# miloknowles/adaptive-stereo-icra-2021

Measured on AMD Instinct MI355X. Metric: stereo pairs/sec (fwd+adapt-step), KITTI 1242x375 D=192, higher is better.
Workload: dtype f32; 1 GPU; KITTI-2015 1242x375, maxdisp 192, k=4 (Dc=12, 24x78 cost volume), forward + one online-adapt step (train-mode BN, monodepth loss, clip 1.0, Adam lr 5e-5); pairs_per_gpu=4, global_batch=4, parallelism=dp1 (per-replica BatchNorm statistics, one flat RCCL gradient all-reduce), kernels=all hand-written HIP (no MIOpen/rocBLAS on the path)

## Files before the change

### adaptive-stereo-icra-2021_amd/adaptive_stereo/_native.py

```python
import ctypes
import os

import torch

_HERE = os.path.dirname(os.path.abspath(__file__))
LIB_PATH = os.path.join(_HERE, "libadaptive_stereo_hip.so")
BUILD_HINT = "build it with: make -C %s" % os.path.join(os.path.dirname(_HERE), "csrc")

c_int, c_float, c_i64, c_vp = ctypes.c_int, ctypes.c_float, ctypes.c_int64, ctypes.c_void_p


class Pcl(ctypes.Structure):
  _fields_ = [(n, ctypes.c_int32) for n in ("B", "D", "H", "W", "pd", "ph", "pw")]

  def numel(self):
    return self.B * (self.D + 2 * self.pd) * (self.H + 2 * self.ph) * (self.W + 2 * self.pw) * 32

  def voxels(self):
    return self.B * self.D * self.H * self.W

  def key(self):
    return (self.B, self.D, self.H, self.W, self.pd, self.ph, self.pw)


# ... 79 lines not shown
                                      c_vp, c_vp, c_vp, c_vp]),
  "as_conv32_wino_bwd_filter": (c_int, [c_vp, c_vp, _P(Pcl), _P(ConvShape), c_vp, c_vp, c_int, c_vp, c_vp]),
  "as_conv32_wino_bwd_parts": (c_int, []),
  "as_conv32_wino_bwd_workspace": (c_i64, []),
  "as_conv32_wino_bwd_generation": (c_int, [c_int]),
  "as_conv32_wino_bwd": (c_int, [c_vp, _P(Pcl), c_vp, c_vp, _P(Pcl), _P(ConvShape), c_vp, c_vp, c_vp, c_vp, c_vp, c_float, c_vp,
                                 c_vp, c_vp, c_vp, c_vp, c_vp, c_vp, c_vp, c_int, c_vp, c_vp, c_vp]),
  "as_conv32_wino_bwd_fused_parts": (c_int, []),
  "as_conv32_wino_bwd_fused_workspace": (c_i64, []),
  "as_conv32_wino_bwd_fused": (c_int, [c_vp, _P(Pcl), c_vp, c_vp, _P(Pcl), _P(ConvShape), c_vp, c_vp, c_vp, c_vp, c_vp, c_float, c_vp,
                                       c_vp, c_vp, c_vp, c_vp, c_vp, c_vp, c_int, c_vp, c_vp, c_vp]),
  "as_conv3d_wgrad_lds_assignment": (c_int, [c_int, c_int, c_int, c_vp, c_vp, c_vp]),
  "as_conv32_s2_enable": (c_int, [c_int]),
  "as_conv4_s2_enable": (c_int, [c_int]),
  "as_conv4_s2_ok": (c_int, [_P(Pcl), _P(Pcl), _P(ConvShape)]),
  "as_conv32_s2_fwd_ok": (c_int, [_P(Pcl), _P(Pcl), _P(ConvShape)]),
  "as_conv32_s2_dgrad_ok": (c_int, [_P(Pcl), _P(Pcl)]),
  "as_conv32_wgrad_segments": (c_int, [_P(Pcl), _P(Pcl), _P(ConvShape)]),
  "as_refine_out_ok": (c_int, [_P(Pcl)]),
  "as_refine_out_fwd": (c_int, [c_vp, c_vp, c_vp, c_vp, c_float, c_vp, _P(Pcl), c_vp, c_vp, c_vp, c_int, c_vp, c_vp]),
  "as_conv32_bwd_fused_ok": (c_int, [_P(Pcl), _P(Pcl), _P(ConvShape)]),
  "as_conv32_bwd_fused_parts": (c_int, []),
  "as_conv32_bwd_fused_workspace": (c_i64, []),
  "as_conv32_bwd_fused": (c_int, [c_vp, _P(Pcl), c_vp, c_vp, _P(Pcl), _P(ConvShape), c_vp, c_vp, c_vp, c_vp, c_vp, c_float, c_vp, c_vp,
                                  c_vp, c_vp, c_vp, c_vp, c_vp, c_int, c_vp, c_vp, c_vp]),
  "as_conv32_bnbwd_parts": (c_int, [_P(Pcl), _P(Pcl), _P(ConvShape)]),
  "as_conv32_fwd_bnbwd": (c_int, [c_vp, _P(Pcl), c_vp, c_vp, _P(Pcl), _P(ConvShape), c_vp, c_vp, c_vp, c_vp, c_vp, c_float,
                                  c_vp, c_vp]),
  "as_agg3d_ok": (c_int, [_P(Pcl)]),
  "as_agg3d_parts": (c_int, [_P(Pcl)]),
  "as_agg3d_plan": (c_int, [_P(Pcl), c_vp]),
  "as_agg3d_fwd": (c_int, [c_vp, _P(Pcl), c_vp, c_vp, c_vp, c_vp, _P(BnMerge), c_vp, c_vp, c_int, c_vp, c_vp, c_float, c_vp, c_vp,
                           c_vp, c_vp]),
  "as_trunk_parts": (c_int, [_P(Pcl), c_int]),
  "as_trunk_fwd": (c_int, [c_vp, c_vp, _P(TrunkBn), c_vp, _P(Pcl), c_int, c_vp, c_vp, c_float, c_vp, c_vp, c_vp, c_vp, c_vp]),
  "as_trunk_finish_fwd": (c_int, [c_vp, _P(Pcl), c_vp, c_vp, c_int, c_int, _P(c_vp), _P(c_vp), c_float, c_vp]),
  "as_trunk_begin_bwd": (c_int, [c_vp, c_vp, c_int, _P(Pcl), c_vp, c_vp]),
  "as_trunk_bwd_workspace": (c_i64, [_P(Pcl), c_int]),
  "as_trunk_bwd": (c_int, [c_vp, c_vp, c_vp, c_vp, c_int, c_vp, c_vp, c_vp, c_vp, c_vp, c_vp, c_vp, c_vp, _P(Pcl), c_int, c_float,
                           c_vp, c_vp, c_int, c_vp, c_vp]),
  "as_trunk_finish_bwd": (c_int, [c_vp, c_int, c_int, _P(c_vp), _P(c_vp), c_int, c_vp]),
  "as_agg_tail_ok": (c_int, [_P(Pcl)]),
  "as_agg_tail_fwd_positions": (c_int, [_P(Pcl)]),
  "as_agg_tail_fwd": (c_int, [c_vp, _P(Pcl), c_vp, c_vp, _P(BnMerge), c_vp, c_vp, c_vp, c_float, c_vp, c_vp, c_vp, c_vp, c_vp]),
  "as_conv3d_out_fwd": (c_int, [c_vp, _P(Pcl), c_vp, c_vp, c_vp, c_vp]),
  "as_conv3d_out_bwd_workspace": (c_i64, [_P(Pcl)]),
  "as_conv3d_out_bwd": (c_int, [c_vp, c_vp, _P(Pcl), c_vp, c_vp, c_vp, c_vp, c_int, c_vp, c_vp]),
  "as_conv32to1_fwd": (c_int, [c_vp, _P(Pcl), _P(ConvShape), c_vp, c_vp, c_vp, c_int, c_vp, c_vp]),
  "as_conv32to1_bwd_workspace": (c_i64, [_P(Pcl), _P(ConvShape)]),
  "as_conv32to1_bwd": (c_int, [c_vp, c_vp, _P(Pcl), _P(ConvShape), c_vp, c_vp, c_vp, c_vp, c_int, c_vp, c_vp]),
  "as_pcl4_numel": (c_i64, [_P(Pcl)]),
  "as_pack_in4": (c_int, [c_vp, c_vp, c_int, c_vp, _P(Pcl), c_vp]),
  "as_conv4_pack_weights": (c_int, [c_vp, c_int, c_vp, _P(ConvShape), c_vp]),
  "as_conv4_wgrad_bnapply_ok": (c_int, [_P(Pcl), _P(Pcl), _P(ConvShape)]),
  "as_conv4_wgrad_bnapply_proj": (c_int, [c_vp, _P(Pcl), c_vp, c_vp, _P(Pcl), _P(ConvShape), c_int, c_vp, c_vp, c_vp, c_vp, c_float,
                                          c_vp, c_vp, c_vp, c_vp, c_int, c_vp, c_vp]),
  "as_tap_gather": (c_int, [c_vp, c_vp, c_vp, c_int, c_int, c_int, c_vp]),
  "as_conv4_wgrad_bnapply": (c_int, [c_vp, _P(Pcl), c_vp, c_vp, _P(Pcl), _P(ConvShape), c_int, c_vp, c_vp, c_vp, c_vp, c_float,
                                     c_vp, c_vp, c_vp, c_int, c_vp, c_vp]),
  "as_conv4_stat_parts": (c_int, [_P(Pcl), _P(Pcl), _P(ConvShape)]),
  "as_conv4_fwd": (c_int, [c_vp, _P(Pcl), c_vp, c_vp, c_vp, _P(Pcl), _P(ConvShape), c_int, c_vp, c_vp, c_float,
                           c_vp, c_vp, c_vp, c_vp]),
  "as_conv4_wgrad_workspace": (c_i64, [_P(Pcl), _P(ConvShape)]),
  "as_conv4_wgrad": (c_int, [c_vp, _P(Pcl), c_vp, _P(Pcl), _P(ConvShape), c_int, c_vp, c_vp, c_int, c_vp, c_vp]),
  "as_softargmax_fwd": (c_int, [c_vp, c_int, c_int, c_int, c_int, c_vp, c_vp, c_vp, c_vp]),
  "as_softargmax_bwd": (c_int, [c_vp, c_vp, c_vp, c_int, c_int, c_int, c_int, c_vp, c_vp]),
# ... 152 lines not shown
```

### adaptive-stereo-icra-2021_amd/adaptive_stereo/hip_ops.py

```python
import torch

from . import _native as nat
from ._native import Pcl, ConvShape, call, ptr, stream, f32c

LEAKY_SLOPE = 0.2
BN_EPS = 1e-5
BN_MOMENTUM = 0.1

CONV3D_333 = ConvShape(3, 3, 3, 1, 1, 1, 1, 1)

_DIRECT_GRADS = True


def set_direct_grad_accumulation(flag: bool):
  global _DIRECT_GRADS
  _DIRECT_GRADS = bool(flag)


def grad_sinks(params):
  if not (_DIRECT_GRADS and torch.is_grad_enabled()):
    return None
  out = []
  for p in params:
    g = getattr(p, "grad", None)
# ... 673 lines not shown

def set_agg3d(flag: bool):
  global _AGG3D
  prev, _AGG3D = _AGG3D, bool(flag)
  return prev


def set_bwd_fused(flag: bool):
  global _BWD_FUSED
  prev, _BWD_FUSED = _BWD_FUSED, bool(flag)
  return prev


_AGG_MERGE_MAX = 512
_TAIL_BWD = True


def set_tail_bwd(flag: bool):
  global _TAIL_BWD
  prev, _TAIL_BWD = _TAIL_BWD, bool(flag)
  return prev


def set_agg_tail(flag: bool):
  global _AGG_TAIL
  prev, _AGG_TAIL = _AGG_TAIL, bool(flag)
  return prev


def agg3d_ok(g: Pcl):
  return _AGG3D and nat.load().as_agg3d_ok(g) == 1


class PendingBn(object):

  def __init__(self, stats: StatParts, gamma, beta, running_mean, running_var):
    self.stats, self.gamma, self.beta, self.rm, self.rv = stats, gamma, beta, running_mean, running_var
    self.state = BnState(gamma.device)
    st = self.state
    self.block = nat.BnMerge(ptr(stats.mean), ptr(stats.m2), ptr(stats.cnt), ptr(gamma), ptr(beta), ptr(running_mean),
                             ptr(running_var), ptr(st.mean), ptr(st.invstd), ptr(st.scale), ptr(st.shift), stats.nparts,
                             BN_MOMENTUM, BN_EPS)

  def finalize(self):
    st = self.state
    with _rmw(self.rm):
      call("as_bn_finalize", ptr(self.stats.mean), ptr(self.stats.m2), ptr(self.stats.cnt), self.stats.nparts, ptr(self.gamma),
           ptr(self.beta), ptr(self.rm), ptr(self.rv), BN_MOMENTUM, BN_EPS, ptr(st.mean), ptr(st.invstd), ptr(st.scale),
           ptr(st.shift), stream())
    return st


def agg3d(x, g: Pcl, packed_w, bias, z=None, in_state=None, in_bn=None, a_out=None, epilogue=0, ep_state=None, stats=None):
  z = z if z is not None else POOL.get(g, x.device)
  sm, s2, sc = (stats.mean, stats.m2, stats.cnt) if stats is not None else (None, None, None)
  with _rmw(in_bn.rm if in_bn is not None else None):
    call("as_agg3d_fwd", ptr(x), g, ptr(packed_w), ptr(bias), ptr(in_state.scale) if in_state is not None else None,
         ptr(in_state.shift) if in_state is not None else None, in_bn.block if in_bn is not None else None, ptr(a_out), ptr(z),
         int(epilogue), ptr(ep_state.scale) if ep_state is not None else None,
         ptr(ep_state.shift) if ep_state is not None else None, LEAKY_SLOPE, ptr(sm), ptr(s2), ptr(sc), stream())
  return z


class CostAggregationFn(torch.autograd.Function):

  @staticmethod
# ... 87 lines not shown
    ctx.mark_non_differentiable(argmax, fcs)
    ctx.set_materialize_grads(False)
    return logits, pred, argmax, fcs

  @staticmethod
  def backward(ctx, g_logits_in, g_pred, _g_argmax, _g_fcs):
    logits, *params = ctx.saved_tensors
    g = ctx.g
    dev = logits.device
    B, D, H, W = logits.shape
    lib = nat.load()
    xs, zs, sts = ctx.xs, ctx.zs, ctx.sts

    g_pred, g_logits_in = f32c(g_pred), f32c(g_logits_in)
    grads = [None] * 18
    w_out = params[16]
    sinks = ctx.sinks
    g_a = POOL.get(g, dev)
    g_wout, g_bout, acc = _grad_dest(_sink(sinks, 16), _sink(sinks, 17), w_out.shape, (1,), dev)
    if not acc:
      grads[16], grads[17] = g_wout, g_bout
    if _TAIL_BWD and lib.as_agg_tail_bwd_ok(g) == 1:
      ws = _empty(lib.as_agg_tail_bwd_workspace(g), dev)
      call("as_agg_tail_bwd", ptr(logits), ptr(g_pred), ptr(g_logits_in), ptr(xs[4]), g, ptr(w_out), ptr(g_a), ptr(g_wout),
           ptr(g_bout), acc, ptr(ws), stream())
    else:
      g_logits = torch.empty_like(logits)
      call("as_softargmax_bwd", ptr(logits), ptr(g_pred), ptr(g_logits_in), B, D, H, W, ptr(g_logits), stream())
      ws = _empty(lib.as_conv3d_out_bwd_workspace(g), dev)
      call("as_conv3d_out_bwd", ptr(g_logits), ptr(xs[4]), g, ptr(w_out), ptr(g_a), ptr(g_wout), ptr(g_bout), acc, ptr(ws),
           stream())

    need_feat = ctx.needs_input_grad[0] or ctx.needs_input_grad[1]
    for l in range(3, -1, -1):
      w, b, gamma, beta = params[4 * l:4 * l + 4]
      g_x, dW, db, g_gamma, g_beta, _ = block_backward(g_a, xs[l], zs[l], sts[l], w, gamma, g, CONV3D_333, ctx.train,
                                                       False, l > 0 or need_feat,
                                                       sinks[4 * l:4 * l + 4] if sinks is not None else None)
      grads[4 * l:4 * l + 4] = [dW, db, g_gamma, g_beta]
      POOL.put(g_a, g); POOL.put(zs[l], g); POOL.put(xs[l + 1], g)
      g_a = g_x
    g_fl = g_fr = None
    if need_feat:
      g_fl = torch.empty(B, 32, H, W, dtype=torch.float32, device=dev)
      g_fr = torch.empty_like(g_fl)
      call("as_cost_volume_bwd", ptr(g_a), ptr(g_fl), ptr(g_fr), g, stream())
      POOL.put(g_a, g)
    POOL.put(xs[0], g)
    ctx.xs = ctx.zs = ctx.sts = None
    return (g_fl, g_fr, None, None, None, None, None) + tuple(grads)


CONV5_S2 = ConvShape(1, 5, 5, 0, 2, 2, 1, 2)


def _down(n):
  return (n - 1) // 2 + 1


_TRUNK = True


def set_trunk(flag: bool):
  global _TRUNK
  prev, _TRUNK = _TRUNK, bool(flag)
  return prev


def trunk_enabled():
  return _TRUNK and _BN_SYNC is None

# ... 677 lines not shown
```

### adaptive-stereo-icra-2021_amd/csrc/agg3d.hip

```cpp
#include "as_common.h"
#include "conv_epilogue.h"
#include "agg3d.h"
#include "bn_merge.h"

#ifndef AGG_WRING
#define AGG_WRING 9
#endif

struct Agg3dArgs {
  const float* x;
  const float* wq;
  const float* in_scale;
  const float* in_shift;
  float* a_out;
  EpilogueArgs ep;
  BnMergeDev in_bn;
  PclDev g;
  int tiles_per_plane, npos, run, groups, slot_bytes;
  int seg_len, nseg, units, per_xcd;
  unsigned wp_magic;
  int strips, Ws, tiles_per_strip;
};

typedef __attribute__((address_space(3))) void* lds_as3_t;

__device__ inline void agg_dma_1kb(const float* sbase, unsigned voff, unsigned m0) {
  asm volatile("s_mov_b32 m0, %0\n\ts_nop 0\n\tglobal_load_lds_dwordx4 %1, %2"
               :: "s"(m0), "v"(voff), "s"(sbase) : "memory", "m0");
}
template <int IMM> __device__ inline void agg_store_imm(float* sbase, unsigned voff, float v) {
  asm volatile("global_store_dword %0, %1, %2 offset:%3" :: "v"(voff), "v"(v), "s"(sbase), "n"(IMM) : "memory");
}
#define AGG_ROW_IMM(r) ((((r) & 3) + 8 * ((r) >> 2)) * 128)
#define AGG_FOR_ROWS(M) M(0) M(1) M(2) M(3) M(4) M(5) M(6) M(7) M(8) M(9) M(10) M(11) M(12) M(13) M(14) M(15)

__device__ inline f32x4 agg_chunk(const char* slot, int v, int h, int q) {
  return *reinterpret_cast<const f32x4*>(slot + v * 128 + (((4 * h + q) ^ ((v >> 1) & 7)) << 4));
}
typedef unsigned agg_u32x4 __attribute__((ext_vector_type(4)));
__device__ inline void agg_load_w(f32x4 (&r)[4], __amdgpu_buffer_rsrc_t rsrc, unsigned lane_bytes, int tap) {
#pragma unroll
  for (int q = 0; q < 4; ++q) {
    const agg_u32x4 v = __builtin_amdgcn_raw_buffer_load_b128(rsrc, lane_bytes + q * 1024, tap * 4096, 0);
    r[q] = __builtin_bit_cast(f32x4, v);
  }
}

__device__ inline int agg_div_wp(int pos, unsigned magic) { return (int)__umulhi((unsigned)pos, magic); }

__device__ inline void agg_issue_plane(const Agg3dArgs& p, int b, int q, int pos0, long plane_vox, unsigned lds0, int wave,
                                       unsigned off_reg, unsigned off_tail, unsigned tail_v0) {
  const float* src = p.x + (((long)b * p.g.Dp + q) * plane_vox + (pos0 - p.g.Wp - 1)) * 32;
  const unsigned slot = lds0 + (unsigned)((q & 3) * p.slot_bytes);
  for (int i = wave; i < p.groups - 1; i += 4)
    agg_dma_1kb(src + i * 256, off_reg, slot + (unsigned)(i * 1024));
  if (((p.groups - 1) & 3) == wave)
    agg_dma_1kb(src + (long)tail_v0 * 32, off_tail, slot + tail_v0 * 128u);
}

__device__ inline void agg_issue_plane_strip(const Agg3dArgs& p, int b, int q, int rs_al, int ng, int xs, unsigned lds0, int wave,
                                             unsigned off_reg) {
  const float* plane = p.x + ((long)b * p.g.Dp + q) * ((long)p.g.Wp * p.g.Hp) * 32;
  const unsigned slot = lds0 + (unsigned)((q & 3) * p.slot_bytes);
  for (int i = wave; i < ng; i += 4) {
    const int pos = rs_al + 8 * i;
    const int y = (int)__umulhi((unsigned)pos, p.wp_magic), xq = pos - y * p.Ws;
    agg_dma_1kb(plane + ((long)y * p.g.Wp + xs + xq) * 32, off_reg, slot + (unsigned)(i * 1024));
  }
}

template <int IN, int EPI, bool STRIP>
__global__ __launch_bounds__(256, 1) void agg3d_kernel(Agg3dArgs p) {
  extern __shared__ __attribute__((aligned(16))) char ring[];
  const unsigned lds0 = __builtin_amdgcn_readfirstlane((unsigned)(unsigned long)((lds_as3_t)ring));
  const int lane = threadIdx.x & 63, wave = __builtin_amdgcn_readfirstlane(threadIdx.x >> 6);
  const int h = lane >> 5, li = lane & 31;
  const int Wp = STRIP ? p.Ws : p.g.Wp;

  const int unit = (blockIdx.x & 7) * p.per_xcd + (blockIdx.x >> 3);
  const bool active = unit < p.units;
  const int col = active ? unit / p.nseg : 0, seg = active ? unit - col * p.nseg : 0;
  const int b = col / p.tiles_per_plane;
  int t = col - b * p.tiles_per_plane;
  const int strip = STRIP ? t / p.tiles_per_strip : 0;
  if (STRIP) t -= strip * p.tiles_per_strip;
  const int xs = STRIP ? min(strip * (p.Ws - 2), p.g.Wp - p.Ws) : 0;
  const int dupc = STRIP ? strip * (p.Ws - 2) - xs : 0;
  const int d0 = seg * p.seg_len, d1 = active ? min(d0 + p.seg_len, p.g.D) : d0;
  const int first = p.g.ph * Wp + p.g.pw;
  const int pos_new = first + 128 * t;
  const int pos0 = min(pos_new, first + p.npos - 128);
  const long plane_vox = (long)p.g.Wp * p.g.Hp;
  const int lead = STRIP ? ((pos0 - Wp - 1) & 7) : 0;
  const int rs_al = pos0 - Wp - 1 - lead;
  const int ng = STRIP ? (lead + 130 + 2 * Wp + 7) >> 3 : p.groups;

  const unsigned vl = (unsigned)(lane >> 3), sl = (unsigned)(lane & 7);
  const unsigned off_reg = vl * 128u + ((sl ^ ((((unsigned)wave & 1u) << 2) | (vl >> 1))) << 4);
  const unsigned tail_v0 = (unsigned)(p.run - 8);
  const unsigned off_tail = vl * 128u + ((sl ^ ((((tail_v0 + vl) >> 1)) & 7u)) << 4);

  auto issue = [&](int q) {
    if (STRIP) agg_issue_plane_strip(p, b, q, rs_al, ng, xs, lds0, wave, off_reg);
    else agg_issue_plane(p, b, q, pos0, plane_vox, lds0, wave, off_reg, off_tail, tail_v0);
  };
  if (active)
    for (int q = d0; q < d0 + 3; ++q) issue(q);

  unsigned keep = 0u, fresh = 0u;
  unsigned so[STRIP ? 16 : 1];
#pragma unroll
  for (int r = 0; r < 16; ++r) {
    const int pos = pos0 + 32 * wave + (r & 3) + 8 * (r >> 2) + 4 * h;
    const int yp = agg_div_wp(pos, p.wp_magic);
    const int xp = pos - yp * Wp;
    bool in = xp >= p.g.pw && xp < p.g.pw + p.g.W;
    bool fr = in && pos >= pos_new;
    if (STRIP) {
      const int gx = xs + xp;
      in = xp >= 1 && xp <= Wp - 2 && gx < p.g.pw + p.g.W;
      fr = in && pos >= pos_new && xp > dupc;
      so[r] = (in ? (unsigned)(yp * p.g.Wp + gx) * 128u : 0u) + 4u * (unsigned)li;
    }
    keep |= (in ? 1u : 0u) << r;
    fresh |= (fr ? 1u : 0u) << r;
  }
  const unsigned io_off = (unsigned)(512 * h + 4 * li);

  f32x4 in_sc = {0.f, 0.f, 0.f, 0.f}, in_sh = {0.f, 0.f, 0.f, 0.f};
  unsigned tmask = 0u, omask = 0u;
  const int cg = threadIdx.x & 7, vrow = threadIdx.x >> 3;
  if (IN == 1) {
    in_sc = *reinterpret_cast<const f32x4*>(p.in_scale + 4 * cg);
    in_sh = *reinterpret_cast<const f32x4*>(p.in_shift + 4 * cg);
  }
  if (IN == 2) {
#ifdef AGG_EXP_NOMERGE
    in_sc = (f32x4){1.f, 1.f, 1.f, 1.f};
#else
    const float* tab = bn_merge_partials<32>(p.in_bn, ring + ((d0 + 3) & 3) * p.slot_bytes, blockIdx.x == 0);
    in_sc = *reinterpret_cast<const f32x4*>(tab + 4 * cg);
    in_sh = *reinterpret_cast<const f32x4*>(tab + 32 + 4 * cg);
    __syncthreads();
#endif
  }
  unsigned ao[STRIP ? 12 : 1];
  if (IN != 0) {
#pragma unroll
    for (int k = 0; k < 12; ++k) {
      const int v = vrow + 32 * k;
      const int pos = rs_al + v;
      const int yp = agg_div_wp(max(pos, 0), p.wp_magic), xp = pos - yp * Wp;
      bool in = v < p.run && xp >= p.g.pw && xp < p.g.pw + p.g.W && yp >= p.g.ph && yp < p.g.ph + p.g.H;
      bool own = in && v >= Wp + 1 && v < Wp + 129;
      if (STRIP) {
        const int gx = xs + xp;
        in = v < 8 * ng && gx >= p.g.pw && gx < p.g.pw + p.g.W && yp >= p.g.ph && yp < p.g.ph + p.g.H;
        own = in && v >= lead + Wp + 1 && v < lead + Wp + 129 && xp >= 1 && xp <= Wp - 2;
        ao[k] = (unsigned)(yp * p.g.Wp + gx) * 128u;
      }
      tmask |= (in ? 1u : 0u) << k;
      omask |= (own ? 1u : 0u) << k;
    }
  }
  char* dump = ring + 4 * p.slot_bytes + threadIdx.x * 16;
  auto activate = [&](int q) {
#ifdef AGG_EXP_NOACT
// ... 1 lines not shown
#endif
    if (q < p.g.pd || q >= p.g.pd + p.g.D) return;
    char* slot = ring + (q & 3) * p.slot_bytes;
    const bool own = p.a_out != nullptr && q - p.g.pd >= d0 && q - p.g.pd < d1;
    float* outp = STRIP ? p.a_out + (((long)b * p.g.Dp + q) * plane_vox) * 32 + 4 * cg
                        : p.a_out + (((long)b * p.g.Dp + q) * plane_vox + (pos0 - Wp - 1)) * 32 + 4 * cg;
    f32x4* cp[12];
    f32x4 y[12];
#pragma unroll
    for (int k = 0; k < 12; ++k) {
      const int v = vrow + 32 * k;
      char* c = slot + v * 128 + ((cg ^ ((v >> 1) & 7)) << 4);
      cp[k] = reinterpret_cast<f32x4*>(((tmask >> k) & 1u) ? c : dump);
      y[k] = *cp[k];
    }
#pragma unroll
    for (int k = 0; k < 12; ++k) {
      y[k].x = fmaf(y[k].x, in_sc.x, in_sh.x); y[k].y = fmaf(y[k].y, in_sc.y, in_sh.y);
      y[k].z = fmaf(y[k].z, in_sc.z, in_sh.z); y[k].w = fmaf(y[k].w, in_sc.w, in_sh.w);
      y[k].x = fmaxf(y[k].x, y[k].x * p.ep.slope); y[k].y = fmaxf(y[k].y, y[k].y * p.ep.slope);
      y[k].z = fmaxf(y[k].z, y[k].z * p.ep.slope); y[k].w = fmaxf(y[k].w, y[k].w * p.ep.slope);
      *cp[k] = y[k];
    }
    if (own) {
#pragma unroll
      for (int k = 0; k < 12; ++k)
        if ((omask >> k) & 1u) {
          if (STRIP) *reinterpret_cast<f32x4*>(reinterpret_cast<char*>(outp) + ao[k]) = y[k];
          else *reinterpret_cast<f32x4*>(outp + (long)(vrow + 32 * k) * 32) = y[k];
        }
    }
  };

  const unsigned wlane = (unsigned)lane * 16u;
  const __amdgpu_buffer_rsrc_t wrsrc = __builtin_amdgcn_make_buffer_rsrc(const_cast<float*>(p.wq), 0, 27 * 4096, 0x00020000);
  const float bias_v = p.ep.bias ? p.ep.bias[li] : 0.f;
  float ep_sc = 1.f, ep_sh = 0.f;
  if (EPI == 1) { ep_sc = p.ep.ep_scale[li]; ep_sh = p.ep.ep_shift[li]; }
  float st_n = 0.f, st_c = 0.f, st_s1 = 0.f, st_s2 = 0.f;

  if (active) {
    asm volatile("s_waitcnt vmcnt(0)" ::: "memory");
    __syncthreads();
    if (IN != 0) {
      for (int q = d0; q < d0 + 3; ++q) activate(q);
      asm volatile("s_waitcnt vmcnt(0)" ::: "memory");
      __syncthreads();
    }
    if (d0 + 1 < d1) issue(d0 + 3);

    f32x4 bw[AGG_WRING][4], a[2][4];
#pragma unroll
    for (int tp = 0; tp < AGG_WRING - 1; ++tp) agg_load_w(bw[tp], wrsrc, wlane, tp);
    const int vbase = lead + 32 * wave + li;

    for (int d = d0; d < d1; ++d) {
      f32x16 acc;
#pragma unroll
      for (int r = 0; r < 16; ++r) acc[r] = bias_v;
      const char* s0 = ring + ((d + 0) & 3) * p.slot_bytes;
      const char* s1 = ring + ((d + 1) & 3) * p.slot_bytes;
      const char* s2 = ring + ((d + 2) & 3) * p.slot_bytes;
#pragma unroll
      for (int q = 0; q < 4; ++q) a[0][q] = agg_chunk(s0, vbase, h, q);
#pragma unroll
      for (int tap = 0; tap < 27; ++tap) {
        agg_load_w(bw[(tap + AGG_WRING - 1) % AGG_WRING], wrsrc, wlane, (tap + AGG_WRING - 1) % 27);
        if (tap + 1 < 27) {
          const int kd = (tap + 1) / 9, tp = (tap + 1) % 9;
          const char* sb = kd == 0 ? s0 : (kd == 1 ? s1 : s2);
          const int v = vbase + (tp / 3) * Wp + (tp % 3);
#pragma unroll
          for (int q = 0; q < 4; ++q) a[(tap + 1) & 1][q] = agg_chunk(sb, v, h, q);
        }
        __builtin_amdgcn_sched_barrier(0);
#pragma unroll
        for (int q = 0; q < 4; ++q) {
          const f32x4 av = a[tap & 1][q], bv = bw[tap % AGG_WRING][q];
          acc = __builtin_amdgcn_mfma_f32_32x32x2f32(av.x, bv.x, acc, 0, 0, 0);
          acc = __builtin_amdgcn_mfma_f32_32x32x2f32(av.y, bv.y, acc, 0, 0, 0);
          acc = __builtin_amdgcn_mfma_f32_32x32x2f32(av.z, bv.z, acc, 0, 0, 0);
          acc = __builtin_amdgcn_mfma_f32_32x32x2f32(av.w, bv.w, acc, 0, 0, 0);
        }
        __builtin_amdgcn_sched_barrier(0);
      }

      if (d + 1 < d1) {
        asm volatile("s_waitcnt vmcnt(%0)" :: "n"(4 * (AGG_WRING - 1)) : "memory");
        __syncthreads();
        if (IN != 0) {
          activate(d + 3);
          __syncthreads();
        }
        if (d + 2 < d1) issue(d + 4);
      }
      __builtin_amdgcn_sched_barrier(0);

      float* z_base = STRIP ? p.ep.z + (((long)b * p.g.Dp + d + p.g.pd) * plane_vox) * 32
                            : p.ep.z + ((((long)b * p.g.Dp + d + p.g.pd) * plane_vox) + pos0 + 32 * wave) * 32;
#define AGG_ST(r) { float v = acc[r];                                                       \
                    if (EPI == 1) { v = fmaf(v, ep_sc, ep_sh); v = v > 0.f ? v : v * p.ep.slope; } \
                    v = ((keep >> r) & 1u) ? v : 0.f;                                        \
                    if (STRIP) agg_store_imm<0>(z_base, so[STRIP ? r : 0], v);               \
                    else agg_store_imm<AGG_ROW_IMM(r)>(z_base, io_off, v); }
      AGG_FOR_ROWS(AGG_ST)
#undef AGG_ST
      if (EPI == 0 && p.ep.stat_mean != nullptr) {
#pragma unroll
        for (int r = 0; r < 16; ++r) {
          const bool f = (fresh >> r) & 1u;
          st_c = (f && st_n == 0.f) ? acc[r] : st_c;
          const float dlt = f ? acc[r] - st_c : 0.f;
          st_s1 += dlt; st_s2 = fmaf(dlt, dlt, st_s2); st_n += f ? 1.f : 0.f;
        }
      }
    }
  }

  if (EPI == 0 && p.ep.stat_mean != nullptr) {
    asm volatile("s_waitcnt vmcnt(0)" ::: "memory");
    __syncthreads();
    float* part = reinterpret_cast<float*>(ring);
    const float mean_l = st_n > 0.f ? st_c + st_s1 / st_n : 0.f;
    const float m2_l = st_n > 0.f ? fmaxf(st_s2 - st_s1 * st_s1 / st_n, 0.f) : 0.f;
    float* mine = part + ((wave * 2 + h) * 32 + li) * 3;
    mine[0] = st_n; mine[1] = mean_l; mine[2] = m2_l;
    __syncthreads();
    if (threadIdx.x < 32) {
      TileStats run; run.n = 0.f; run.mean = 0.f; run.m2 = 0.f;
      for (int q = 0; q < 8; ++q) {
        TileStats ts;
        ts.n = part[(q * 32 + li) * 3]; ts.mean = part[(q * 32 + li) * 3 + 1]; ts.m2 = part[(q * 32 + li) * 3 + 2];
        stats_merge(run, ts);
      }
      stats_write(p.ep, blockIdx.x, run);
    }
  }
}

#define AGG_MAX_WP 83
static int agg_strips(const as_pcl* g) { return g->W + 2 <= AGG_MAX_WP ? 1 : as_div_up(g->W, 78); }
static int agg_ws(const as_pcl* g) {
  const int n = agg_strips(g);
  if (n == 1) return g->W + 2;
  return (as_div_up(g->W, n) + 2 + 7) / 8 * 8;
}
static int agg_run(const as_pcl* g) { return 130 + 2 * agg_ws(g) + (agg_strips(g) > 1 ? 7 : 0); }
static int agg_tiles_per_strip(const as_pcl* g) {
// ... 80 lines not shown
  AS_CHECK_ARG(epilogue != 1 || (ep_scale && ep_shift), "as_agg3d_fwd: epilogue 1 needs scale and shift");
  AS_CHECK_ARG((in_scale == nullptr) == (in_shift == nullptr), "as_agg3d_fwd: in_scale and in_shift must pair");
  AS_CHECK_ARG(!(in_scale && in_bn), "as_agg3d_fwd: pass the input BatchNorm either as an affine or as partials, not both");
  AS_CHECK_ARG(a_out == nullptr || in_scale != nullptr || in_bn != nullptr, "as_agg3d_fwd: a_out needs the input BatchNorm");
  AS_CHECK_ARG((in_scale == nullptr && in_bn == nullptr) || epilogue == 0, "as_agg3d_fwd: an input BatchNorm goes with epilogue 0");
  AS_CHECK_ARG((stat_mean == nullptr) == (stat_m2 == nullptr) && (stat_mean == nullptr) == (stat_cnt == nullptr),
               "as_agg3d_fwd: the three moment buffers must pair");
  AS_CHECK_ARG(a_out == nullptr || a_out != x, "as_agg3d_fwd: a_out must not alias the input");
  Agg3dArgs a;
  a.x = x; a.wq = packed_w; a.in_scale = in_scale; a.in_shift = in_shift; a.a_out = a_out;
  if (in_bn) AS_CHECK_ARG(bn_merge_fill(&a.in_bn, in_bn), "as_agg3d_fwd: incomplete as_bn_merge block");
  a.ep.bias = bias; a.ep.z = z; a.ep.ep_scale = ep_scale; a.ep.ep_shift = ep_shift; a.ep.residual = nullptr;
  const bool moments = epilogue == 0 && stat_mean != nullptr;
  a.ep.stat_mean = moments ? stat_mean : nullptr; a.ep.stat_m2 = moments ? stat_m2 : nullptr;
  a.ep.stat_cnt = moments ? stat_cnt : nullptr;
  a.ep.epilogue = epilogue; a.ep.slope = slope;
  a.g = as_make_dev(g);
  agg_fill_plan(g, a);
  const int lds_bytes = 4 * a.slot_bytes + 4096;
  hipStream_t st = (hipStream_t)stream;
  const double flops = 2.0 * (double)g->B * g->D * g->H * g->W * 1024.0 * 27.0;
  as_prof_mark(7, st, 1, 0.0);
  int e;
  if (in_bn) e = agg_launch_t<2, 0>(a, lds_bytes, st);
  else if (in_scale) e = agg_launch_t<1, 0>(a, lds_bytes, st);
  else if (epilogue == 1) e = agg_launch_t<0, 1>(a, lds_bytes, st);
  else if (moments) e = agg_launch_t<0, 0>(a, lds_bytes, st);
  else e = agg_launch_t<0, 2>(a, lds_bytes, st);
  if (e) return e;
  as_prof_mark(7, st, 0, flops);
  AS_CHECK_LAUNCH("as_agg3d_fwd");
  return AS_OK;
}
```

### adaptive-stereo-icra-2021_amd/csrc/as_common.h

```cpp
#pragma once
#include <hip/hip_runtime.h>
#include <stdint.h>
#include <stdio.h>
#include <stdarg.h>

#include "../../include/adaptive_stereo_hip.h"

#define AS_OK 0
#define AS_ERR_ARG (-1)
#define AS_ERR_LAUNCH (-2)

void as_set_error(const char* fmt, ...);
void as_wgrad_reduce_enqueue(hipStream_t st, const float* partial, const float* partial_db, int nchunks, int T, float* dW,
                             float* db, int accumulate);
#define AS_CURSOR_MAX_BATCH 65535
void as_cursor_advance_enqueue(hipStream_t st, int32_t* cursor, int32_t* dropped, int B, int capacity);
void as_zero_i32_enqueue(hipStream_t st, int32_t* p, int n);
void as_prof_mark(int kernel_id, hipStream_t st, int begin, double flops);
enum {
  AS_PROF_CONV32 = 0, AS_PROF_WGRAD32 = 1, AS_PROF_CONV32_LDS = 2, AS_PROF_WGRAD32_LDS = 3, AS_PROF_BN_ACT_FWD = 4,
  AS_PROF_BN_BWD = 5, AS_PROF_CONV32_LDS_BNBWD = 6, AS_PROF_AGG3D = 7, AS_PROF_AGG_TAIL = 8, AS_PROF_WGRAD3D_LDS = 9,
  AS_PROF_COSTVOL_FWD = 10, AS_PROF_COSTVOL_BWD = 11, AS_PROF_OUTCONV_BWD = 12, AS_PROF_SOFTARGMAX_BWD = 13,
  AS_PROF_UPSAMPLE_FWD = 14, AS_PROF_UPSAMPLE_BWD = 15, AS_PROF_WARP_FWD = 16, AS_PROF_WARP_BWD = 17,
  AS_PROF_LOSS_FWD = 18, AS_PROF_LOSS_BWD = 19, AS_PROF_OUTCONV_FWD = 20, AS_PROF_SOFTARGMAX_FWD = 21, AS_PROF_BWD_FUSED = 22, AS_PROF_CONV_ACT = 23,
  AS_PROF_WINO_DGRAD = 24, AS_PROF_WINO_WGRAD = 25, AS_PROF_WINO_FWD = 26,
  AS_PROF_WINO_BWD = 27,
  AS_PROF_IDS = 28
};

#define AS_CHECK_ARG(cond, ...)            \
  do {                                     \
    if (!(cond)) {                         \
      as_set_error(__VA_ARGS__);           \
      return AS_ERR_ARG;                   \
    }                                      \
  } while (0)

#define AS_CHECK_LAUNCH(name)                                              \
  do {                                                                     \
    hipError_t e_ = hipGetLastError();                                     \
    if (e_ != hipSuccess) {                                                \
      as_set_error("%s: launch failed: %s", name, hipGetErrorString(e_));  \
      return AS_ERR_LAUNCH;                                                \
    }                                                                      \
  } while (0)

typedef float f32x4 __attribute__((ext_vector_type(4)));
typedef float f32x16 __attribute__((ext_vector_type(16)));

struct PclDev {
  int B, D, H, W;
  int pd, ph, pw;
  int Dp, Hp, Wp;
  __host__ __device__ inline long vox(int b, int d, int y, int x) const {
    return (((long)b * Dp + d + pd) * Hp + y + ph) * (long)Wp + x + pw;
  }
};

static inline PclDev as_make_dev(const as_pcl* g) {
  PclDev p;
// ... 79 lines not shown
```

### include/adaptive_stereo_hip.h

```cpp
#ifndef ADAPTIVE_STEREO_HIP_H_
#define ADAPTIVE_STEREO_HIP_H_

#include <stdint.h>

#ifdef __cplusplus
extern "C" {
#endif

#define AS_CHANNELS 32
#define AS_MAX_TAPS 32

typedef struct as_pcl {
  int32_t B, D, H, W;
  int32_t pd, ph, pw;
} as_pcl;

typedef struct as_conv_shape {
  int32_t kd, kh, kw;
  int32_t pad_d, pad_h, pad_w;
  int32_t dil;
  int32_t stride;
} as_conv_shape;

const char* as_last_error(void);
// ... 85 lines not shown
int as_conv4_s2_ok(const as_pcl* gin, const as_pcl* gout, const as_conv_shape* s);
int as_conv32_s2_fwd_ok(const as_pcl* gin, const as_pcl* gout, const as_conv_shape* s);
int as_conv32_s2_dgrad_ok(const as_pcl* ggz, const as_pcl* ggx);
int as_conv32_wgrad_segments(const as_pcl* gin, const as_pcl* gout, const as_conv_shape* s);

int as_refine_out_ok(const as_pcl* g);
int as_refine_out_fwd(const float* x, const float* skip, const float* scale, const float* shift, float slope, float* a_out,
                      const as_pcl* g, const float* w, const float* bias, const float* add_src, int relu, float* out,
                      void* stream);

typedef struct as_bn_merge {
  const float* stat_mean;
  const float* stat_m2;
  const float* stat_cnt;
  const float* gamma;
  const float* beta;
  float* running_mean;
  float* running_var;
  float* save_mean;
  float* save_invstd;
  float* scale;
  float* shift;
  int32_t nparts;
  float momentum;
  float eps;
} as_bn_merge;
int as_agg3d_ok(const as_pcl* g);
int as_agg3d_parts(const as_pcl* g);
int as_agg3d_plan(const as_pcl* g, int out[8]);
int as_agg3d_fwd(const float* x, const as_pcl* g, const float* packed_w, const float* bias,
                 const float* in_scale, const float* in_shift, const as_bn_merge* in_bn, float* a_out,
                 float* z, int epilogue, const float* ep_scale, const float* ep_shift, float slope,
                 float* stat_mean, float* stat_m2, float* stat_cnt, void* stream);

int as_agg_tail_ok(const as_pcl* g);
int as_agg_tail_fwd_positions(const as_pcl* g);
int as_agg_tail_fwd(const float* x, const as_pcl* g, const float* in_scale, const float* in_shift,
                    const as_bn_merge* in_bn, float* a_out,
                    const float* w, const float* bias, float slope, float* logits, float* pred,
                    int32_t* argmax, float* fcs, void* stream);

typedef struct as_trunk_bn {
  const float* stat_mean;
  const float* stat_m2;
  const float* stat_cnt;
  const float* gamma;
  const float* beta;
  float* state;
  int32_t nparts;
  float eps;
} as_trunk_bn;
int as_trunk_parts(const as_pcl* g, int ngroups);
int as_trunk_fwd(const float* src, const float* skip, const as_trunk_bn* bn_prev, float* a_out, const as_pcl* g, int ngroups,
                 const float* packed_w, const float* bias, float slope, float* z, float* stat_mean, float* stat_m2,
                 float* stat_cnt, void* stream);
int as_trunk_finish_fwd(const float* feats_pcl, const as_pcl* g, float* feats_nchw, const float* states, int nlayers,
                        int ngroups, float* const* running_mean, float* const* running_var, float momentum, void* stream);
int as_trunk_begin_bwd(const float* g_a, const float* g_b, int nA, const as_pcl* g, float* out_pcl, void* stream);
int64_t as_trunk_bwd_workspace(const as_pcl* g, int ngroups);
int as_trunk_bwd(const float* g_a, const float* z, const float* state, const double* sums, int nparts, const float* gamma,
                 float* bn_grads, const float* x, const float* packed_wt, float* g_x, const float* z_next,
                 const float* state_next, double* sums_next, const as_pcl* g, int ngroups, float slope, float* dW, float* db,
                 int accumulate, float* workspace, void* stream);
int as_trunk_finish_bwd(const float* bn_grads, int nlayers, int ngroups, float* const* g_gamma, float* const* g_beta,
                        int accumulate, void* stream);

// ... 291 lines not shown
```

Baseline: 607.8 stereo pairs/s.

## Fuse BN/LeakyReLU backward into agg3d dgrad conv with next-layer BN sums

Adds a backward mode to the 3D aggregation conv kernel (IN==3). It applies the BN+LeakyReLU backward to the incoming gradient on the fly as it loads each depth slice into LDS, and writes g_z as a by-product. An EPI==3 epilogue also accumulates the lower layer's BN backward reductions (sum dy, sum dy*xhat) into per-block partials. The goal is to remove the separate BN-backward elementwise pass and the separate reduction pass for each 3D aggregation layer. The cost is extra z loads, more register pressure in the conv kernel, and a path limited to single-strip geometries without synced BN.

```diff
diff --git a/adaptive-stereo-icra-2021_amd/adaptive_stereo/_native.py b/adaptive-stereo-icra-2021_amd/adaptive_stereo/_native.py
--- a/adaptive-stereo-icra-2021_amd/adaptive_stereo/_native.py
+++ b/adaptive-stereo-icra-2021_amd/adaptive_stereo/_native.py
@@ -135,6 +135,10 @@
   "as_agg3d_plan": (c_int, [_P(Pcl), c_vp]),
   "as_agg3d_fwd": (c_int, [c_vp, _P(Pcl), c_vp, c_vp, c_vp, c_vp, _P(BnMerge), c_vp, c_vp, c_int, c_vp, c_vp, c_float, c_vp, c_vp,
                            c_vp, c_vp]),
+  "as_agg3d_bwd_fused_ok": (c_int, [_P(Pcl)]),
+  "as_agg3d_bwd_fused_parts": (c_int, [_P(Pcl)]),
+  "as_agg3d_bwd_fused": (c_int, [c_vp, c_vp, _P(Pcl), c_vp, c_vp, c_vp, c_vp, c_vp, c_float, c_vp, c_vp, c_vp, c_vp, c_vp, c_vp,
+                                 c_vp, c_vp]),
   "as_trunk_parts": (c_int, [_P(Pcl), c_int]),
   "as_trunk_fwd": (c_int, [c_vp, c_vp, _P(TrunkBn), c_vp, _P(Pcl), c_int, c_vp, c_vp, c_float, c_vp, c_vp, c_vp, c_vp, c_vp]),
   "as_trunk_finish_fwd": (c_int, [c_vp, _P(Pcl), c_vp, c_vp, c_int, c_int, _P(c_vp), _P(c_vp), c_float, c_vp]),
diff --git a/adaptive-stereo-icra-2021_amd/adaptive_stereo/hip_ops.py b/adaptive-stereo-icra-2021_amd/adaptive_stereo/hip_ops.py
--- a/adaptive-stereo-icra-2021_amd/adaptive_stereo/hip_ops.py
+++ b/adaptive-stereo-icra-2021_amd/adaptive_stereo/hip_ops.py
@@ -729,6 +729,40 @@
   return _AGG3D and nat.load().as_agg3d_ok(g) == 1
 
 
+_AGG3D_BWD_FUSED = True
+
+
+def set_agg3d_bwd_fused(flag: bool):
+  global _AGG3D_BWD_FUSED
+  prev, _AGG3D_BWD_FUSED = _AGG3D_BWD_FUSED, bool(flag)
+  return prev
+
+
+def agg3d_bwd_fused_ok(g: Pcl):
+  return _AGG3D_BWD_FUSED and agg3d_ok(g) and _BN_SYNC is None and nat.load().as_agg3d_bwd_fused_ok(g) == 1
+
+
+def agg3d_block_backward(g_out, x, z, st, w, gamma, g: Pcl, train, sinks=None, sums=None, next_bn=None):
+  lib = nat.load()
+  dev = z.device
+  sw, sb, sg, sbeta = sinks if sinks is not None else (None, None, None, None)
+  ws = sums.workspace if sums is not None else _empty(lib.as_bn_bwd_workspace(g), dev)
+  g_gamma, g_beta, acc = _grad_dest(sg, sbeta, (32,), (32,), dev)
+  bn_bwd_coefs(g_out, z, st, gamma, g, train, g_gamma, g_beta, acc, ws, sums)
+  coef = ws[lib.as_bn_bwd_coef_offset():]
+  g_z, g_x = POOL.get(g, dev), POOL.get(g, dev)
+  next_z, next_st = next_bn if next_bn is not None else (None, None)
+  nws = _empty(lib.as_bn_bwd_workspace(g), dev) if next_bn is not None else None
+  call("as_agg3d_bwd_fused", ptr(g_out), ptr(z), g, ptr(pack_weights(w, CONV3D_333, True)), ptr(st.scale), ptr(st.shift),
+       ptr(st.mean), ptr(coef), LEAKY_SLOPE, ptr(g_z), ptr(g_x), ptr(next_z),
+       ptr(next_st.scale) if next_st is not None else None, ptr(next_st.shift) if next_st is not None else None,
+       ptr(next_st.mean) if next_st is not None else None, ptr(nws), stream())
+  dW, db = conv32_wgrad(x, g, g_z, g, CONV3D_333, True, sw, sb)
+  POOL.put(g_z, g)
+  next_sums = BnBwdSums(nws, lib.as_agg3d_bwd_fused_parts(g)) if next_bn is not None else None
+  return g_x, dW, db, (None if acc else g_gamma), (None if acc else g_beta), next_sums
+
+
 class PendingBn(object):
 
   def __init__(self, stats: StatParts, gamma, beta, running_mean, running_var):
@@ -882,11 +916,18 @@
            stream())
 
     need_feat = ctx.needs_input_grad[0] or ctx.needs_input_grad[1]
+    sums = None
     for l in range(3, -1, -1):
       w, b, gamma, beta = params[4 * l:4 * l + 4]
-      g_x, dW, db, g_gamma, g_beta, _ = block_backward(g_a, xs[l], zs[l], sts[l], w, gamma, g, CONV3D_333, ctx.train,
-                                                       False, l > 0 or need_feat,
-                                                       sinks[4 * l:4 * l + 4] if sinks is not None else None)
+      lsinks = sinks[4 * l:4 * l + 4] if sinks is not None else None
+      if (l > 0 or need_feat) and zs[l] is not None and agg3d_bwd_fused_ok(g):
+        next_bn = (zs[l - 1], sts[l - 1]) if l > 0 and zs[l - 1] is not None else None
+        g_x, dW, db, g_gamma, g_beta, sums = agg3d_block_backward(g_a, xs[l], zs[l], sts[l], w, gamma, g, ctx.train, lsinks,
+                                                                  sums, next_bn)
+      else:
+        g_x, dW, db, g_gamma, g_beta, _ = block_backward(g_a, xs[l], zs[l], sts[l], w, gamma, g, CONV3D_333, ctx.train,
+                                                         False, l > 0 or need_feat, lsinks, sums=sums)
+        sums = None
       grads[4 * l:4 * l + 4] = [dW, db, g_gamma, g_beta]
       POOL.put(g_a, g); POOL.put(zs[l], g); POOL.put(xs[l + 1], g)
       g_a = g_x
diff --git a/adaptive-stereo-icra-2021_amd/csrc/agg3d.hip b/adaptive-stereo-icra-2021_amd/csrc/agg3d.hip
--- a/adaptive-stereo-icra-2021_amd/csrc/agg3d.hip
+++ b/adaptive-stereo-icra-2021_amd/csrc/agg3d.hip
@@ -20,6 +20,14 @@
   int seg_len, nseg, units, per_xcd;
   unsigned wp_magic;
   int strips, Ws, tiles_per_strip;
+  const float* bz;
+  const float* b_mean;
+  const float* b_coef;
+  const float* nz;
+  const float* n_scale;
+  const float* n_shift;
+  const float* n_mean;
+  double* n_partial;
 };
 
 typedef __attribute__((address_space(3))) void* lds_as3_t;
@@ -71,6 +79,7 @@
 
 template <int IN, int EPI, bool STRIP>
 __global__ __launch_bounds__(256, 1) void agg3d_kernel(Agg3dArgs p) {
+  static_assert(IN != 3 || !STRIP, "IN 3 exists in the contiguous form only");
   extern __shared__ __attribute__((aligned(16))) char ring[];
   const unsigned lds0 = __builtin_amdgcn_readfirstlane((unsigned)(unsigned long)((lds_as3_t)ring));
   const int lane = threadIdx.x & 63, wave = __builtin_amdgcn_readfirstlane(threadIdx.x >> 6);
@@ -130,9 +139,16 @@
   f32x4 in_sc = {0.f, 0.f, 0.f, 0.f}, in_sh = {0.f, 0.f, 0.f, 0.f};
   unsigned tmask = 0u, omask = 0u;
   const int cg = threadIdx.x & 7, vrow = threadIdx.x >> 3;
-  if (IN == 1) {
+  if (IN == 1 || IN == 3) {
     in_sc = *reinterpret_cast<const f32x4*>(p.in_scale + 4 * cg);
     in_sh = *reinterpret_cast<const f32x4*>(p.in_shift + 4 * cg);
+  }
+  f32x4 b_mu = {0.f, 0.f, 0.f, 0.f}, b_k1 = b_mu, b_k2 = b_mu, b_k3 = b_mu;
+  if (IN == 3) {
+    b_mu = *reinterpret_cast<const f32x4*>(p.b_mean + 4 * cg);
+    b_k1 = *reinterpret_cast<const f32x4*>(p.b_coef + 4 * cg);
+    b_k2 = *reinterpret_cast<const f32x4*>(p.b_coef + 32 + 4 * cg);
+    b_k3 = *reinterpret_cast<const f32x4*>(p.b_coef + 64 + 4 * cg);
   }
   if (IN == 2) {
 #ifdef AGG_EXP_NOMERGE
@@ -200,22 +216,81 @@
     }
   };
 
+  auto zfetch = [&](int q, f32x4 (&zr)[12]) {
+    if (q < p.g.pd || q >= p.g.pd + p.g.D) return;
+    const float* zp = p.bz + (((long)b * p.g.Dp + q) * plane_vox + (pos0 - Wp - 1)) * 32 + 4 * cg;
+#pragma unroll
+    for (int k = 0; k < 12; ++k) {
+      const int v = ((tmask >> k) & 1u) ? vrow + 32 * k : vrow;
+      zr[k] = *reinterpret_cast<const f32x4*>(zp + v * 32);
+    }
+  };
+  auto bwd_apply = [&](int q, const f32x4 (&zr)[12]) {
+    if (q < p.g.pd || q >= p.g.pd + p.g.D) return;
+    char* slot = ring + (q & 3) * p.slot_bytes;
+    const bool own = p.a_out != nullptr && q - p.g.pd >= d0 && q - p.g.pd < d1;
+    float* outp = p.a_out + (((long)b * p.g.Dp + q) * plane_vox + (pos0 - Wp - 1)) * 32 + 4 * cg;
+    f32x4* cp[12];
+    f32x4 y[12];
+#pragma unroll
+    for (int k = 0; k < 12; ++k) {
+      const int v = vrow + 32 * k;
+      char* c = slot + v * 128 + ((cg ^ ((v >> 1) & 7)) << 4);
+      cp[k] = reinterpret_cast<f32x4*>(((tmask >> k) & 1u) ? c : dump);
+      y[k] = *cp[k];
+    }
+#pragma unroll
+    for (int k = 0; k < 12; ++k) {
+      f32x4 o;
+#pragma unroll
+      for (int i = 0; i < 4; ++i) {
+        const float zz = zr[k][i], gy = y[k][i];
+        const float yy = __builtin_fmaf(zz, in_sc[i], in_sh[i]);
+        const float gs = gy * p.ep.slope;
+        const float gg = yy > 0.f ? gy : gs;
+        const float t = gg - b_k1[i];
+        const float xc = zz - b_mu[i];
+        o[i] = __builtin_fmaf(-b_k2[i], xc, t) * b_k3[i];
+      }
+      y[k] = o;
+      *cp[k] = o;
+    }
+    if (own) {
+#pragma unroll
+      for (int k = 0; k < 12; ++k)
+        if ((omask >> k) & 1u) *reinterpret_cast<f32x4*>(outp + (long)(vrow + 32 * k) * 32) = y[k];
+    }
+  };
+
   const unsigned wlane = (unsigned)lane * 16u;
   const __amdgpu_buffer_rsrc_t wrsrc = __builtin_amdgcn_make_buffer_rsrc(const_cast<float*>(p.wq), 0, 27 * 4096, 0x00020000);
   const float bias_v = p.ep.bias ? p.ep.bias[li] : 0.f;
   float ep_sc = 1.f, ep_sh = 0.f;
   if (EPI == 1) { ep_sc = p.ep.ep_scale[li]; ep_sh = p.ep.ep_shift[li]; }
   float st_n = 0.f, st_c = 0.f, st_s1 = 0.f, st_s2 = 0.f;
+  float n_sc = 0.f, n_sh = 0.f, n_mu = 0.f, s_dy = 0.f, s_dx = 0.f;
+  if (EPI == 3) { n_sc = p.n_scale[li]; n_sh = p.n_shift[li]; n_mu = p.n_mean[li]; }
+  f32x4 zr[12] = {};
 
   if (active) {
+    f32x4 z0[IN == 3 ? 12 : 1] = {}, z1[IN == 3 ? 12 : 1] = {};
+    if constexpr (IN == 3) { zfetch(d0, z0); zfetch(d0 + 1, z1); zfetch(d0 + 2, zr); }
     asm volatile("s_waitcnt vmcnt(0)" ::: "memory");
     __syncthreads();
-    if (IN != 0) {
+    if (IN == 1 || IN == 2) {
       for (int q = d0; q < d0 + 3; ++q) activate(q);
       asm volatile("s_waitcnt vmcnt(0)" ::: "memory");
       __syncthreads();
     }
-    if (d0 + 1 < d1) issue(d0 + 3);
+    if constexpr (IN == 3) {
+      bwd_apply(d0, z0); bwd_apply(d0 + 1, z1); bwd_apply(d0 + 2, zr);
+      asm volatile("s_waitcnt vmcnt(0)" ::: "memory");
+      __syncthreads();
+    }
+    if (d0 + 1 < d1) {
+      issue(d0 + 3);
+      if (IN == 3) zfetch(d0 + 3, zr);
+    }
 
     f32x4 bw[AGG_WRING][4], a[2][4];
 #pragma unroll
@@ -226,6 +301,12 @@
       f32x16 acc;
 #pragma unroll
       for (int r = 0; r < 16; ++r) acc[r] = bias_v;
+      float nzv[EPI == 3 ? 16 : 1];
+      if (EPI == 3) {
+        const char* nzb = reinterpret_cast<const char*>(p.nz + ((((long)b * p.g.Dp + d + p.g.pd) * plane_vox) + pos0 + 32 * wave) * 32) + io_off;
+#pragma unroll
+        for (int r = 0; r < 16; ++r) nzv[EPI == 3 ? r : 0] = *reinterpret_cast<const float*>(nzb + AGG_ROW_IMM(r));
+      }
       const char* s0 = ring + ((d + 0) & 3) * p.slot_bytes;
       const char* s1 = ring + ((d + 1) & 3) * p.slot_bytes;
       const char* s2 = ring + ((d + 2) & 3) * p.slot_bytes;
@@ -256,11 +337,18 @@
       if (d + 1 < d1) {
         asm volatile("s_waitcnt vmcnt(%0)" :: "n"(4 * (AGG_WRING - 1)) : "memory");
         __syncthreads();
-        if (IN != 0) {
+        if (IN == 1 || IN == 2) {
           activate(d + 3);
           __syncthreads();
         }
-        if (d + 2 < d1) issue(d + 4);
+        if (IN == 3) {
+          bwd_apply(d + 3, zr);
+          __syncthreads();
+        }
+        if (d + 2 < d1) {
+          issue(d + 4);
+          if (IN == 3) zfetch(d + 4, zr);
+        }
       }
       __builtin_amdgcn_sched_barrier(0);
 
@@ -282,6 +370,30 @@
           st_s1 += dlt; st_s2 = fmaf(dlt, dlt, st_s2); st_n += f ? 1.f : 0.f;
         }
       }
+      if (EPI == 3) {
+#pragma unroll
+        for (int r = 0; r < 16; ++r) {
+          const float zz = nzv[EPI == 3 ? r : 0];
+          const float gy = __builtin_fmaf(zz, n_sc, n_sh) > 0.f ? acc[r] : acc[r] * p.ep.slope;
+          const float gf = ((fresh >> r) & 1u) ? gy : 0.f;
+          s_dy += gf; s_dx = fmaf(gf, zz - n_mu, s_dx);
+        }
+      }
+    }
+  }
+
+  if (EPI == 3) {
+    asm volatile("s_waitcnt vmcnt(0)" ::: "memory");
+    __syncthreads();
+    double* part = reinterpret_cast<double*>(ring);
+    part[(wave * 2 + h) * 64 + li] = (double)s_dy;
+    part[(wave * 2 + h) * 64 + 32 + li] = (double)s_dx;
+    __syncthreads();
+    if (threadIdx.x < 64) {
+      double s = 0.0;
+#pragma unroll
+      for (int q = 0; q < 8; ++q) s += part[q * 64 + threadIdx.x];
+      p.n_partial[(long)blockIdx.x * 64 + threadIdx.x] = s;
     }
   }
 
@@ -428,3 +540,46 @@
   AS_CHECK_LAUNCH("as_agg3d_fwd");
   return AS_OK;
 }
+
+#define AGG_BWD_MAX_PARTS 1024
+static bool agg3d_bwd_fused_applicable(const as_pcl* g) {
+  return agg3d_applicable(g) && agg_strips(g) == 1 && agg3d_units(g) <= AGG_BWD_MAX_PARTS;
+}
+extern "C" int as_agg3d_bwd_fused_ok(const as_pcl* g) { return agg3d_bwd_fused_applicable(g) ? 1 : 0; }
+extern "C" int as_agg3d_bwd_fused_parts(const as_pcl* g) { return agg3d_bwd_fused_applicable(g) ? agg3d_units(g) : 0; }
+
+extern "C" int as_agg3d_bwd_fused(const float* g_a, const float* z, const as_pcl* g, const float* packed_w_t,
+                                  const float* scale, const float* shift, const float* mean, const float* coef, float slope,
+                                  float* g_z, float* g_x, const float* next_z, const float* next_scale,
+                                  const float* next_shift, const float* next_mean, float* next_workspace, void* stream) {
+  AS_CHECK_ARG(agg3d_bwd_fused_applicable(g), "as_agg3d_bwd_fused: geometry not supported (as_agg3d_bwd_fused_ok() == 0)");
+  AS_CHECK_ARG(g_a && z && packed_w_t && scale && shift && mean && coef && g_z && g_x, "as_agg3d_bwd_fused: null pointer");
+  const bool sums = next_workspace != nullptr;
+  AS_CHECK_ARG(!sums || (next_z && next_scale && next_shift && next_mean),
+               "as_agg3d_bwd_fused: the lower layer's sums need its z, scale, shift and mean");
+  AS_CHECK_ARG(!sums || ((uintptr_t)next_workspace & 7) == 0, "as_agg3d_bwd_fused: next_workspace must be 8-byte aligned");
+  const int64_t bytes = (int64_t)g->B * (g->D + 2) * (g->H + 2) * (g->W + 2) * 128;
+  const AsRange r[] = {{g_a, bytes}, {z, bytes}, {next_z, bytes}, {g_z, bytes}, {g_x, bytes},
+                       {next_workspace, (int64_t)agg3d_units(g) * 64 * 8}};
+  AS_CHECK_ARG(as_disjoint(r, 3, 6), "as_agg3d_bwd_fused: g_z, g_x and next_workspace must not overlap an input or each other");
+  Agg3dArgs a;
+  a.x = g_a; a.wq = packed_w_t; a.in_scale = scale; a.in_shift = shift; a.a_out = g_z;
+  a.in_bn = BnMergeDev();
+  a.ep.bias = nullptr; a.ep.z = g_x; a.ep.ep_scale = nullptr; a.ep.ep_shift = nullptr; a.ep.residual = nullptr;
+  a.ep.stat_mean = nullptr; a.ep.stat_m2 = nullptr; a.ep.stat_cnt = nullptr;
+  a.ep.epilogue = 2; a.ep.slope = slope;
+  a.bz = z; a.b_mean = mean; a.b_coef = coef;
+  a.nz = next_z; a.n_scale = next_scale; a.n_shift = next_shift; a.n_mean = next_mean;
+  a.n_partial = reinterpret_cast<double*>(next_workspace);
+  a.g = as_make_dev(g);
+  agg_fill_plan(g, a);
+  const int lds_bytes = 4 * a.slot_bytes + 4096;
+  hipStream_t st = (hipStream_t)stream;
+  const double flops = 2.0 * (double)g->B * g->D * g->H * g->W * 1024.0 * 27.0;
+  as_prof_mark(AS_PROF_AGG3D_BWD, st, 1, 0.0);
+  const int e = sums ? agg_launch_s<3, 3, false>(a, lds_bytes, st) : agg_launch_s<3, 2, false>(a, lds_bytes, st);
+  if (e) return e;
+  as_prof_mark(AS_PROF_AGG3D_BWD, st, 0, flops);
+  AS_CHECK_LAUNCH("as_agg3d_bwd_fused");
+  return AS_OK;
+}
diff --git a/adaptive-stereo-icra-2021_amd/csrc/as_common.h b/adaptive-stereo-icra-2021_amd/csrc/as_common.h
--- a/adaptive-stereo-icra-2021_amd/csrc/as_common.h
+++ b/adaptive-stereo-icra-2021_amd/csrc/as_common.h
@@ -25,7 +25,8 @@
   AS_PROF_LOSS_FWD = 18, AS_PROF_LOSS_BWD = 19, AS_PROF_OUTCONV_FWD = 20, AS_PROF_SOFTARGMAX_FWD = 21, AS_PROF_BWD_FUSED = 22, AS_PROF_CONV_ACT = 23,
   AS_PROF_WINO_DGRAD = 24, AS_PROF_WINO_WGRAD = 25, AS_PROF_WINO_FWD = 26,
   AS_PROF_WINO_BWD = 27,
-  AS_PROF_IDS = 28
+  AS_PROF_AGG3D_BWD = 28,
+  AS_PROF_IDS = 29
 };
 
 #define AS_CHECK_ARG(cond, ...)            \
diff --git a/include/adaptive_stereo_hip.h b/include/adaptive_stereo_hip.h
--- a/include/adaptive_stereo_hip.h
+++ b/include/adaptive_stereo_hip.h
@@ -141,6 +141,13 @@
                  const float* in_scale, const float* in_shift, const as_bn_merge* in_bn, float* a_out,
                  float* z, int epilogue, const float* ep_scale, const float* ep_shift, float slope,
                  float* stat_mean, float* stat_m2, float* stat_cnt, void* stream);
+
+int as_agg3d_bwd_fused_ok(const as_pcl* g);
+int as_agg3d_bwd_fused_parts(const as_pcl* g);
+int as_agg3d_bwd_fused(const float* g_a, const float* z, const as_pcl* g, const float* packed_w_t,
+                       const float* scale, const float* shift, const float* mean, const float* coef, float slope,
+                       float* g_z, float* g_x, const float* next_z, const float* next_scale, const float* next_shift,
+                       const float* next_mean, float* next_workspace, void* stream);
 
 int as_agg_tail_ok(const as_pcl* g);
 int as_agg_tail_fwd_positions(const as_pcl* g);
```

Measured after the change: 602.5 stereo pairs/s. About the same (-0.9%).
